# sebastian-hofstaetter/matchmaker

Hardware: NVIDIA H100
Metric: query-doc pairs scored/sec (ColBERT max-sim d=128) (higher is better)
Workload: dtype f16

## Files before the change

### matchmaker_b200/csrc/maxsim_qm.cu

```cuda
#include <cuda_bf16.h>
#include <cuda_fp16.h>

#include <algorithm>

#include "device_util.cuh"
#include "host_util.cuh"
#include "masks.cuh"
#include "maxsim.cuh"
#include "ptx.cuh"

namespace mmb {

namespace {

constexpr int kThreads = 384;
constexpr int kChunkRows = 64;
constexpr int kChunkKBlockBytes = kChunkRows * 128;
constexpr int kMaxStages = 32;
constexpr int kMaxLd = 4096;
constexpr int kScouts = 3;
constexpr int kRecordStep = 6;
constexpr int kMaxRecords = 48;
constexpr int kRecordReserve = 12 * 1024;
constexpr int kQSlots = 2;
constexpr int kQRows = 32;
constexpr int kQBlockBytes = kQRows * 128;
constexpr uint32_t kFill = 1u << 16, kLiveMask = kFill - 1;
constexpr int kRecBits = 4;
constexpr int kRegsHelper = 120, kRegsConsumer = 192;

#ifdef MMB200_ENABLE_PROF
enum QmProf {
  kPrTotal, kPrQEmpty, kPrRFull, kPrEmpty, kPrTma, kPrChunks,
  kCoTotal, kCoRFull, kCoFull, kCoIssue, kCoMma, kCoReduce, kCoEpilogue, kCoDocs,
  kScTotal, kScREmpty,
  kProfCount
};
__device__ unsigned long long g_qm_prof[kProfCount];
#define QM_PROF(...) __VA_ARGS__
#else
#define QM_PROF(...)
#endif

struct QmShared {
  uint64_t full[kMaxStages];
  uint64_t empty[kMaxStages];
  uint64_t qfull[kQSlots];
  uint64_t qempty[kQSlots];
  uint64_t rfull[kMaxRecords];
  uint64_t rempty[kMaxRecords];
  float xm[2][2][4][32];
  int32_t xa[2][2][4][32];
};

struct QmLaunch {
  int32_t kblocks;
  int32_t stages;
  int32_t chunk_bytes;
  int32_t records;
  int32_t rec_words;
};

struct RecCursor {
  int slot;
  uint32_t phase;
  __device__ __forceinline__ void advance(int step, int records) {
    slot += step;
    if (slot >= records) { slot -= records; phase ^= 1u; }
  }
};

struct QmMaps {
  CUtensorMap q;
  CUtensorMap d;
};

template <bool kStore>
struct PairStream {
  struct Batch {
    int32_t q, d, dm, rows;
    int64_t row0, row_end;
  };
  const MaxsimParams& P;
  int64_t first, end, step;
  int64_t pre_batch;
  int k;
  int lane;
  Batch cur, nxt, pre;

  __device__ __forceinline__ PairStream(const MaxsimParams& P_, int64_t first_, int64_t end_, int64_t step_, int lane_)
      : P(P_), first(first_), end(end_), step(step_), lane(lane_) {
    load1(cur, 0);
    load1(nxt, 1);
    load2(cur);
    load2(nxt);
    resolve(cur);
    pre_batch = 2;
    load1(pre, pre_batch);
    k = -1;
  }
  __device__ __forceinline__ void load1(Batch& b, int64_t bi) {
    const int64_t p = first + (bi * 32 + lane) * step;
    b.q = 0; b.d = -1; b.dm = 0; b.rows = 0; b.row0 = 0; b.row_end = 0;
    if (p >= end) return;
    b.q = P.pair_q ? P.pair_q[p] : (int32_t)((p + P.pair_base) / P.docs_per_query);
    b.d = P.pair_d ? P.pair_d[p] : (int32_t)p;
    if (P.pair_dmask) b.dm = P.pair_dmask[p];
  }
  __device__ __forceinline__ void load2(Batch& b) {
    if (!P.pair_dmask) b.dm = b.d;
    if constexpr (kStore) {
      if (b.d >= 0) { b.row0 = P.doc_offsets[b.d]; b.row_end = P.doc_offsets[b.d + 1]; }
    }
  }
  __device__ __forceinline__ void resolve(Batch& b) {
    if constexpr (kStore) b.rows = (int)max((int64_t)0, min(b.row_end - b.row0, (int64_t)P.Ld));
  }
  __device__ __forceinline__ void next() {
    if (++k == 32) {
      cur = nxt;
      resolve(cur);
      nxt = pre;
      load2(nxt);
      load1(pre, ++pre_batch);
      k = 0;
    }
  }
  __device__ __forceinline__ int64_t q() const { return __shfl_sync(0xffffffffu, cur.q, k); }
  __device__ __forceinline__ int64_t d() const { return __shfl_sync(0xffffffffu, cur.d, k); }
  __device__ __forceinline__ int64_t dm() const { return __shfl_sync(0xffffffffu, cur.dm, k); }
  __device__ __forceinline__ int rows() const { return __shfl_sync(0xffffffffu, cur.rows, k); }
  __device__ __forceinline__ int64_t row0() const { return __shfl_sync(0xffffffffu, cur.row0, k); }
};

template <typename T>
__device__ __forceinline__ void wgmma_n32(float (&d)[16], uint64_t a, uint64_t b, uint32_t acc);
template <>
__device__ __forceinline__ void wgmma_n32<__half>(float (&d)[16], uint64_t a, uint64_t b, uint32_t acc) {
  wgmma_m64n32k16_f16(d, a, b, acc);
}
template <>
__device__ __forceinline__ void wgmma_n32<__nv_bfloat16>(float (&d)[16], uint64_t a, uint64_t b, uint32_t acc) {
  wgmma_m64n32k16_bf16(d, a, b, acc);
}

template <bool kArgmax>
__device__ __forceinline__ void take(float v, int row, float& m, int& am) {
  if constexpr (kArgmax) {
    const bool gt = v > m;
    m = gt ? v : m;
    am = gt ? row : am;
  } else {
    m = fmaxf(m, v);
  }
}

template <typename T, bool kArgmax, bool kStore>
__global__ void __launch_bounds__(kThreads, 1)
maxsim_qm_kernel(const __grid_constant__ QmMaps M, MaxsimParams P, QmLaunch L) {
  extern __shared__ uint8_t smem_raw[];
  uint8_t* smem = smem_raw + ((1024u - (smem_u32(smem_raw) & 1023u)) & 1023u);
  const int qslot_bytes = L.kblocks * kQBlockBytes;
  uint8_t* q_base = smem;
  uint8_t* stage_base = q_base + kQSlots * qslot_bytes;
  uint32_t* rec_base = reinterpret_cast<uint32_t*>(stage_base + (size_t)L.stages * L.chunk_bytes);
  QmShared* S = reinterpret_cast<QmShared*>(rec_base + (size_t)L.records * L.rec_words);

  const int warp = threadIdx.x >> 5;
  const int lane = threadIdx.x & 31;

  int64_t p_begin, p_end;
  cta_share(P.n_pairs, &p_begin, &p_end);

  if (threadIdx.x == 0) {
    prefetch_tensormap(&M.q);
    prefetch_tensormap(&M.d);
    for (int s = 0; s < L.stages; ++s) { mbar_init(&S->full[s], 1); mbar_init(&S->empty[s], 4); }
    for (int s = 0; s < kQSlots; ++s) { mbar_init(&S->qfull[s], 1); mbar_init(&S->qempty[s], 8); }
    for (int r = 0; r < L.records; ++r) {
      mbar_init(&S->rfull[r], 1);
      mbar_init(&S->rempty[r], 5);
      rec_base[(size_t)r * L.rec_words + kRecBits - 2] = 0;
      rec_base[(size_t)r * L.rec_words + kRecBits - 1] = 0;
    }
    fence_barrier_init();
  }
  __syncthreads();

  if (warp == 0) {
    setmaxnreg_dec<kRegsHelper>();
    PairStream<kStore> meta(P, p_begin, p_end, 1, lane);
    const int ring = L.stages >> 1;
    int st_cur = 0, st_oth = 0;
    uint32_t ph_cur = 0, ph_oth = 0;
    int64_t prev_q = -1;
    uint32_t qcount = 0;
    RecCursor rc{0, 0};
    QM_PROF(unsigned long long prof[kProfCount] = {}; const long long t_start = clock64(); long long t_;)
    for (int64_t p = p_begin; p < p_end; ++p) {
      meta.next();
      const int64_t qi = meta.q();
      const int64_t di = meta.d();
      const int64_t row0 = kStore ? meta.row0() : 0;
      if (qi != prev_q) {
        const uint32_t slot = qcount & 1u, use = qcount >> 1;
        QM_PROF(t_ = clock64();)
        mbar_wait(&S->qempty[slot], (use & 1u) ^ 1u);
        QM_PROF(prof[kPrQEmpty] += clock64() - t_;)
        if (elect_one_sync()) {
          mbar_arrive_expect_tx(&S->qfull[slot], (uint32_t)(L.kblocks * kQBlockBytes));
          for (int kb = 0; kb < L.kblocks; ++kb)
            tma_load_4d(&M.q, q_base + (size_t)slot * qslot_bytes + kb * kQBlockBytes, &S->qfull[slot], 0, 0, kb, (int)qi,
                        kEvictLast);
        }
        __syncwarp();
        ++qcount;
        prev_q = qi;
      }
      const int c = (int)((p - p_begin) & 1);
      QM_PROF(t_ = clock64();)
      mbar_wait(&S->rfull[rc.slot], rc.phase);
      QM_PROF(prof[kPrRFull] += clock64() - t_;)
      const int live = (int)(rec_base[(size_t)rc.slot * L.rec_words] & kLiveMask);
      __syncwarp();
      if (lane == 0) mbar_arrive(&S->rempty[rc.slot]);
      rc.advance(1, L.records);
      const int dcoord = kStore ? 0 : (int)di;
      const int nch = max(1, (live + kChunkRows - 1) / kChunkRows);
      int row = kStore ? (int)row0 : live - kChunkRows * nch;
      for (int ch = 0; ch < nch; ++ch, row += kChunkRows) {
        const int stage = c * ring + st_cur;
        QM_PROF(t_ = clock64();)
        mbar_wait(&S->empty[stage], ph_cur ^ 1u);
        QM_PROF(prof[kPrEmpty] += clock64() - t_; t_ = clock64(); ++prof[kPrChunks];)
        if (elect_one_sync()) {
          if (live == 0) {
            mbar_arrive(&S->full[stage]);
          } else {
            mbar_arrive_expect_tx(&S->full[stage], (uint32_t)L.chunk_bytes);
            tma_load_4d(&M.d, stage_base + (size_t)stage * L.chunk_bytes, &S->full[stage], 0, row, 0, dcoord, kEvictFirst);
          }
        }
        __syncwarp();
        QM_PROF(prof[kPrTma] += clock64() - t_;)
        if (++st_cur == ring) { st_cur = 0; ph_cur ^= 1u; }
      }
      const int st = st_cur; st_cur = st_oth; st_oth = st;
      const uint32_t ph = ph_cur; ph_cur = ph_oth; ph_oth = ph;
    }
    QM_PROF(prof[kPrTotal] = clock64() - t_start;
            if (lane == 0) for (int i = kPrTotal; i <= kPrChunks; ++i) atomicAdd(&g_qm_prof[i], prof[i]);)
  } else if (warp <= kScouts) {
    setmaxnreg_dec<kRegsHelper>();
    constexpr int kW = 8;
    const int s = warp - 1;
    const int dmt = P.d_mask ? P.mask_dtype : MMB200_MASK_NONE;
    const int nwin = (P.Ld + 32 * kW - 1) / (32 * kW);
    const int bit_words = L.rec_words - kRecBits;
    PairStream<kStore> meta(P, p_begin + s, p_end, kScouts, lane);
    RecCursor rc{s, 0};
    int64_t fp = p_begin + s;
    auto load_win = [&](uint32_t (&raw)[kW], int64_t dm, int w) {
#pragma unroll
      for (int k = 0; k < kW; ++k) {
        const int g = w * 32 * kW + 32 * k + lane;
        raw[k] = 1;
        if (dmt != MMB200_MASK_NONE && g < P.Ld) {
          const uint64_t v = mask_raw(P.d_mask, dmt, dm * (int64_t)P.Ld + g);
          raw[k] = (uint32_t)(v | (v >> 32));
        }
      }
    };
    auto fetch = [&](uint32_t (&raw)[kW], int64_t& dm, int& lim) {
      if (fp < p_end) {
        meta.next();
        dm = meta.dm();
        lim = kStore ? meta.rows() : P.Ld;
        load_win(raw, dm, 0);
      }
      fp += kScouts;
    };
    QM_PROF(unsigned long long prof_re = 0; const long long t_start = clock64();)
    auto doc = [&](uint32_t (&raw)[kW], int64_t& dm, int& lim) {
      QM_PROF(const long long t_ = clock64();)
      mbar_wait(&S->rempty[rc.slot], rc.phase ^ 1u);
      QM_PROF(prof_re += clock64() - t_;)
      uint32_t* rec = rec_base + (size_t)rc.slot * L.rec_words;
      int live = 0;
      bool masked = false;
      for (int w = 0; w < nwin; ++w) {
        if (w > 0) load_win(raw, dm, w);
#pragma unroll
        for (int k = 0; k < kW; ++k) {
          const int g = w * 32 * kW + 32 * k + lane;
          const bool in_doc = g < lim;
          const bool ok = in_doc && mask_test(raw[k], dmt);
          masked |= in_doc && !ok;
          const uint32_t b = __ballot_sync(0xffffffffu, ok);
          const int wi = w * kW + k;
          if (b) live = 32 * wi + 32 - __clz(b);
          if (lane == 0 && wi < bit_words) rec[kRecBits + wi] = b;
        }
      }
      const bool fill = !kStore && __any_sync(0xffffffffu, masked);
      fetch(raw, dm, lim);
      if (lane == 0) {
        rec[0] = (uint32_t)live | (fill ? kFill : 0u);
        mbar_arrive(&S->rfull[rc.slot]);
      }
      rc.advance(kScouts, L.records);
    };
    uint32_t ra[kW], rb[kW];
    int64_t dma = 0, dmb = 0;
    int la = 0, lb = 0;
    fetch(ra, dma, la);
    fetch(rb, dmb, lb);
    for (int64_t sp = p_begin + s; sp < p_end;) {
      doc(ra, dma, la);
      if ((sp += kScouts) >= p_end) break;
      doc(rb, dmb, lb);
      sp += kScouts;
    }
    QM_PROF(if (lane == 0) {
      atomicAdd(&g_qm_prof[kScTotal], (unsigned long long)(clock64() - t_start));
      atomicAdd(&g_qm_prof[kScREmpty], prof_re);
    })
  } else {
    setmaxnreg_inc<kRegsConsumer>();
    const int c = (warp >> 2) - 1;
    const int wq = warp & 3;
    const int r0 = 16 * wq + (lane >> 2);
    const int qmt = P.q_mask ? P.mask_dtype : MMB200_MASK_NONE;
    const int ring = L.stages >> 1;
    int64_t prev_q = -1;
    uint32_t qcount = 0;
    int cur_slot = 0;
    RecCursor rc{c, 0};
    auto load_q = [&](int64_t n0) -> int32_t { return p_begin + n0 + lane < p_end ? P.pair_q[p_begin + n0 + lane] : 0; };
    int32_t qb_cur = 0, qb_nxt = 0;
    if (P.pair_q) { qb_cur = load_q(0); qb_nxt = load_q(32); }
    int64_t q_run = 0;
    int32_t q_rem = 0;
    if (!P.pair_q) {
      q_run = (p_begin + P.pair_base) / P.docs_per_query;
      q_rem = (int32_t)((p_begin + P.pair_base) - q_run * P.docs_per_query);
    }
    QM_PROF(unsigned long long prof[kProfCount] = {}; const long long t_start = clock64(); long long t_;)
    int64_t n_walk = 0;
    auto walk_to = [&](int64_t n) {
      for (; n_walk <= n; ++n_walk) {
        int64_t qi;
        if (P.pair_q) {
          if ((n_walk & 31) == 0 && n_walk > 0) { qb_cur = qb_nxt; qb_nxt = load_q(n_walk + 32); }
          qi = __shfl_sync(0xffffffffu, qb_cur, (int)(n_walk & 31));
        } else {
          qi = q_run;
          if (++q_rem == P.docs_per_query) { q_rem = 0; ++q_run; }
        }
        if (qi != prev_q) {
          if (prev_q >= 0) { __syncwarp(); if (lane == 0) mbar_arrive(&S->qempty[cur_slot]); }
          cur_slot = (int)(qcount & 1u);
          mbar_wait(&S->qfull[cur_slot], (qcount >> 1) & 1u);
          ++qcount;
          prev_q = qi;
        }
      }
      return prev_q;
    };
    struct Doc {
      int64_t n;
      uint32_t qlo;
      uint64_t qraw;
      int slot;
      uint32_t head;
      int live, nch;
    };
    auto begin = [&](Doc& D, int64_t n) {
      const int64_t qi = walk_to(n);
      D.n = n;
      D.qlo = (uint32_t)make_wgmma_sw128_desc(smem_u32(q_base + (size_t)cur_slot * qslot_bytes));
      D.qraw = 0;
      if (wq == 0 && lane < P.Lq)
        D.qraw = (qmt != MMB200_MASK_NONE) ? mask_raw(P.q_mask, qmt, qi * (int64_t)P.Lq + lane) : 1;
      QM_PROF(t_ = clock64();)
      mbar_wait(&S->rfull[rc.slot], rc.phase);
      QM_PROF(prof[kCoRFull] += clock64() - t_; ++prof[kCoDocs];)
      D.slot = rc.slot;
      rc.advance(2, L.records);
      D.head = rec_base[(size_t)D.slot * L.rec_words];
      D.live = (int)(D.head & kLiveMask);
      D.nch = max(1, (D.live + kChunkRows - 1) / kChunkRows);
    };
    int st_next = 0;
    uint32_t ph_next = 0;
    constexpr uint64_t kDescHi = (uint64_t)(1024 >> 4) << 32 | (uint64_t)1 << 62;
    auto issue = [&](float (&acc)[16], uint32_t qlo_doc) -> int {
      const int stage = c * ring + st_next;
      QM_PROF(t_ = clock64();)
      mbar_wait(&S->full[stage], ph_next);
      QM_PROF(prof[kCoFull] += clock64() - t_; t_ = clock64();)
      if (++st_next == ring) { st_next = 0; ph_next ^= 1u; }
      const uint32_t daddr = smem_u32(stage_base + (size_t)stage * L.chunk_bytes);
      const uint32_t dlo = (uint32_t)make_wgmma_sw128_desc(__shfl_sync(0xffffffffu, daddr, 0));
      const uint32_t qlo = __shfl_sync(0xffffffffu, qlo_doc, 0);
      wgmma_fence();
#pragma unroll
      for (int k = 0; k < 4; ++k) wgmma_n32<T>(acc, kDescHi | (dlo + 2 * k), kDescHi | (qlo + 2 * k), k != 0);
      if (L.kblocks > 1) {
#pragma unroll
        for (int k = 0; k < 4; ++k)
          wgmma_n32<T>(acc, kDescHi | (dlo + (kChunkKBlockBytes >> 4) + 2 * k),
                       kDescHi | (qlo + (kQBlockBytes >> 4) + 2 * k), 1);
      }
      wgmma_commit();
      wgmma_fence_regs(acc);
      QM_PROF(prof[kCoIssue] += clock64() - t_;)
      return stage;
    };
    float mx[8];
    int ax[8];
#pragma unroll
    for (int e = 0; e < 8; ++e) { mx[e] = -INFINITY; ax[e] = -1; }
    auto reduce = [&](float (&acc)[16], int stage, const Doc& D, int ch) {
      wgmma_fence_regs(acc);
      const int col0 = kStore ? kChunkRows * ch : D.live - kChunkRows * (D.nch - ch);
      const int x0 = col0 + r0, x1 = x0 + 8;
      const uint32_t* bits = rec_base + (size_t)D.slot * L.rec_words + kRecBits;
      const float p0 = (bits[x0 >> 5] >> (x0 & 31)) & 1u ? 0.f : -INFINITY;
      const float p1 = (bits[x1 >> 5] >> (x1 & 31)) & 1u ? 0.f : -INFINITY;
#pragma unroll
      for (int e = 0; e < 8; ++e) {
        const int i = 4 * (e >> 1) + (e & 1);
        take<kArgmax>(acc[i] + p0, x0, mx[e], ax[e]);
        take<kArgmax>(acc[i + 2] + p1, x1, mx[e], ax[e]);
      }
      __syncwarp();
      if (lane == 0) mbar_arrive(&S->empty[stage]);
    };
    auto combine = [&](float om, int oa, float& m, int& a) {
      if constexpr (kArgmax) {
        if (om > m || (om == m && (unsigned)oa < (unsigned)a)) { m = om; a = oa; }
      } else {
        m = fmaxf(m, om);
      }
    };
    auto epilogue = [&](const Doc& D) {
      QM_PROF(t_ = clock64();)
      if (lane == 0) mbar_arrive(&S->rempty[D.slot]);
#pragma unroll
      for (int o = 4; o < 32; o <<= 1) {
#pragma unroll
        for (int e = 0; e < 8; ++e) {
          const float om = __shfl_xor_sync(0xffffffffu, mx[e], o);
          const int oa = kArgmax ? __shfl_xor_sync(0xffffffffu, ax[e], o) : 0;
          combine(om, oa, mx[e], ax[e]);
        }
      }
      const int buf = (int)((D.n >> 1) & 1);
      float* xm = S->xm[c][buf][0];
      int32_t* xa = S->xa[c][buf][0];
      if (lane < 4) {
#pragma unroll
        for (int e = 0; e < 8; ++e) {
          const int t = 8 * (e >> 1) + 2 * lane + (e & 1);
          xm[32 * wq + t] = mx[e];
          if constexpr (kArgmax) xa[32 * wq + t] = ax[e];
        }
      }
#pragma unroll
      for (int e = 0; e < 8; ++e) { mx[e] = -INFINITY; ax[e] = -1; }
      if (wq != 0) {
        named_bar_arrive(1 + c, 128);
      } else {
        named_bar_sync(1 + c, 128);
        float m = xm[lane];
        int a = kArgmax ? xa[lane] : -1;
#pragma unroll
        for (int w = 1; w < 4; ++w) combine(xm[32 * w + lane], kArgmax ? xa[32 * w + lane] : 0, m, a);
        if (D.head & kFill) take<kArgmax>(-1000.f, P.Ld, m, a);
        const bool ok = mask_test(D.qraw, qmt);
        const int64_t p = p_begin + D.n;
        if constexpr (kArgmax) {
          if (lane < P.Lq) P.argmax[p * (int64_t)P.Lq + lane] = (ok && a < P.Ld) ? a : -1;
        }
        float s = ok ? m : 0.f;
        s += __shfl_down_sync(0xffffffffu, s, 8);
#pragma unroll
        for (int o = 1; o < 8; o <<= 1) s += __shfl_xor_sync(0xffffffffu, s, o);
        const float hi = __shfl_sync(0xffffffffu, s, 16);
        if (lane == 0) P.out[p] = s + hi;
      }
      QM_PROF(prof[kCoEpilogue] += clock64() - t_;)
    };
    const int64_t n_pairs = p_end - p_begin;
    float acc[16];
    for (int64_t n = c; n < n_pairs; n += 2) {
      Doc D;
      begin(D, n);
      for (int ch = 0; ch < D.nch; ++ch) {
        const int st = issue(acc, D.qlo);
        QM_PROF(t_ = clock64();)
        wgmma_wait<0>();
        QM_PROF(prof[kCoMma] += clock64() - t_; t_ = clock64();)
        reduce(acc, st, D, ch);
        QM_PROF(prof[kCoReduce] += clock64() - t_;)
      }
      epilogue(D);
    }
    QM_PROF(prof[kCoTotal] = clock64() - t_start;
            if (wq == 0 && lane == 0) for (int i = kCoTotal; i <= kCoDocs; ++i) atomicAdd(&g_qm_prof[i], prof[i]);)
  }
}

template <typename T, bool kArgmax, bool kStore>
int launch_qm(int grid, size_t smem_bytes, cudaStream_t stream, const QmMaps& M, const MaxsimParams& P,
              const QmLaunch& L) {
  MMB_CHECK_CUDA(cudaFuncSetAttribute(maxsim_qm_kernel<T, kArgmax, kStore>, cudaFuncAttributeMaxDynamicSharedMemorySize,
                                      (int)smem_bytes));
  maxsim_qm_kernel<T, kArgmax, kStore><<<grid, kThreads, smem_bytes, stream>>>(M, P, L);
  MMB_CHECK_CUDA(cudaGetLastError());
  return MMB200_OK;
}

int launch_qm_dispatch(int grid, size_t smem_bytes, cudaStream_t stream, const QmMaps& M, const MaxsimParams& P,
                       const QmLaunch& L, int dtype) {
  if (P.doc_offsets)
    return dtype == MMB200_F16 ? launch_qm<__half, false, true>(grid, smem_bytes, stream, M, P, L)
                               : launch_qm<__nv_bfloat16, false, true>(grid, smem_bytes, stream, M, P, L);
  if (dtype == MMB200_F16)
    return P.argmax ? launch_qm<__half, true, false>(grid, smem_bytes, stream, M, P, L)
                    : launch_qm<__half, false, false>(grid, smem_bytes, stream, M, P, L);
  return P.argmax ? launch_qm<__nv_bfloat16, true, false>(grid, smem_bytes, stream, M, P, L)
                  : launch_qm<__nv_bfloat16, false, false>(grid, smem_bytes, stream, M, P, L);
}

}

int maxsim_qm_launch(const MaxsimParams& P, int dtype, const DeviceInfo& dev, cudaStream_t stream, bool* handled) {
  *handled = false;
  if (dtype != MMB200_F16 && dtype != MMB200_BF16) return MMB200_OK;
  if (P.Lq > kQRows || (P.dim != 64 && P.dim != 128) || P.Ld > kMaxLd) return MMB200_OK;
  if ((reinterpret_cast<uintptr_t>(P.q) | reinterpret_cast<uintptr_t>(P.d)) & 15) return MMB200_OK;
  if (P.doc_offsets && P.argmax) return MMB200_OK;
  QmLaunch L;
  L.kblocks = P.dim / 64;
  L.chunk_bytes = L.kblocks * kChunkKBlockBytes;
  L.rec_words = kRecBits + 2 * ((P.Ld + kChunkRows - 1) / kChunkRows);
  const int fixed = kQSlots * L.kblocks * kQBlockBytes + (int)sizeof(QmShared) + 1024;
  L.stages = std::min(kMaxStages, (dev.max_smem_optin - fixed - kRecordReserve) / L.chunk_bytes) & ~1;
  const int rec_bytes = L.rec_words * 4;
  L.records = std::min(kMaxRecords, (dev.max_smem_optin - fixed - L.stages * L.chunk_bytes) / rec_bytes);
  L.records -= L.records % kRecordStep;
  if (L.stages < 4 || L.records < kRecordStep) return MMB200_OK;
  const size_t smem_bytes = (size_t)L.stages * L.chunk_bytes + (size_t)L.records * rec_bytes + fixed;

  const CUtensorMapDataType tdt = dtype == MMB200_F16 ? CU_TENSOR_MAP_DATA_TYPE_FLOAT16 : CU_TENSOR_MAP_DATA_TYPE_BFLOAT16;
  QmMaps M;
  {
    const uint64_t dims[4] = {64, (uint64_t)P.Lq, (uint64_t)L.kblocks, (uint64_t)P.n_q};
    const uint64_t strides[3] = {(uint64_t)P.dim * 2, 128, (uint64_t)P.Lq * P.dim * 2};
    const uint32_t box[4] = {64, (uint32_t)kQRows, 1, 1};
    if (int rc = encode_tensor_map(&M.q, tdt, 4, P.q, dims, strides, box, CU_TENSOR_MAP_SWIZZLE_128B,
                                   CU_TENSOR_MAP_L2_PROMOTION_L2_128B))
      return rc;
  }
  const uint64_t d_rows = P.doc_offsets ? (uint64_t)P.n_rows : (uint64_t)P.Ld;
  const uint64_t d_count = P.doc_offsets ? 1 : (uint64_t)P.n_d;
  {
    const uint64_t dims[4] = {64, d_rows, (uint64_t)L.kblocks, d_count};
    const uint64_t strides[3] = {(uint64_t)P.dim * 2, 128, d_rows * P.dim * 2};
    const uint32_t box[4] = {64, (uint32_t)kChunkRows, (uint32_t)L.kblocks, 1};
    if (int rc = encode_tensor_map(&M.d, tdt, 4, P.d, dims, strides, box, CU_TENSOR_MAP_SWIZZLE_128B,
                                   CU_TENSOR_MAP_L2_PROMOTION_L2_256B))
      return rc;
  }
  *handled = true;
  const int grid = (int)std::min<int64_t>(dev.sm_count, P.n_pairs);
#ifdef MMB200_ENABLE_PROF
  const bool prof = getenv("MMB200_MAXSIM_PROF") != nullptr;
  if (prof) {
    const unsigned long long zero[kProfCount] = {};
    MMB_CHECK_CUDA(cudaMemcpyToSymbolAsync(g_qm_prof, zero, sizeof(zero), 0, cudaMemcpyHostToDevice, stream));
  }
  const int rc = launch_qm_dispatch(grid, smem_bytes, stream, M, P, L, dtype);
  if (prof && rc == MMB200_OK) {
    unsigned long long h[kProfCount];
    MMB_CHECK_CUDA(cudaMemcpyFromSymbolAsync(h, g_qm_prof, sizeof(h), 0, cudaMemcpyDeviceToHost, stream));
    MMB_CHECK_CUDA(cudaStreamSynchronize(stream));
    const double ctas = grid, wgs = 2.0 * grid, scouts = (double)kScouts * grid;
    const double chunks = (double)h[kPrChunks], docs = (double)h[kCoDocs];
    fprintf(stderr,
            "maxsim_prof pairs %lld Ld %d chunks %.0f | cycles per CTA: producer total %.0f qempty %.0f rfull %.0f "
            "empty %.0f tma %.0f | per consumer warpgroup: total %.0f rfull %.0f full %.0f issue %.0f mma %.0f "
            "reduce %.0f epilogue %.0f | per scout: total %.0f rempty %.0f | per chunk: producer %.0f (empty %.0f, "
            "tma %.0f), warpgroup full %.0f issue %.0f mma %.0f reduce %.0f | per document per warpgroup: total %.0f "
            "epilogue %.0f rfull %.0f\n",
            (long long)P.n_pairs, P.Ld, chunks, h[kPrTotal] / ctas, h[kPrQEmpty] / ctas, h[kPrRFull] / ctas,
            h[kPrEmpty] / ctas, h[kPrTma] / ctas, h[kCoTotal] / wgs, h[kCoRFull] / wgs, h[kCoFull] / wgs,
            h[kCoIssue] / wgs, h[kCoMma] / wgs, h[kCoReduce] / wgs, h[kCoEpilogue] / wgs, h[kScTotal] / scouts,
            h[kScREmpty] / scouts, h[kPrTotal] / chunks, h[kPrEmpty] / chunks, h[kPrTma] / chunks, h[kCoFull] / chunks,
            h[kCoIssue] / chunks, h[kCoMma] / chunks, h[kCoReduce] / chunks, h[kCoTotal] / docs, h[kCoEpilogue] / docs,
            h[kCoRFull] / docs);
  }
  return rc;
#else
  return launch_qm_dispatch(grid, smem_bytes, stream, M, P, L, dtype);
#endif
}

}
```

Before: 145.6 million.

## Use three consumer warpgroups instead of two in maxsim kernel

Raises the CTA from 384 to 512 threads so three consumer warpgroups take pairs round-robin. The stage ring is split three ways, the producer rotates over three stage cursors, and record stepping and barrier counts are adjusted to match. The intent is more concurrent MMA and reduction work per SM to hide epilogue and wait latency. In exchange, consumer registers drop from 192 to 128 per thread and there are fewer stages per consumer ring, which could cause spills or starve the pipeline.

```diff
diff --git a/matchmaker_b200/csrc/maxsim_qm.cu b/matchmaker_b200/csrc/maxsim_qm.cu
--- a/matchmaker_b200/csrc/maxsim_qm.cu
+++ b/matchmaker_b200/csrc/maxsim_qm.cu
@@ -13,27 +13,29 @@
 
 namespace {
 
-constexpr int kThreads = 384;
+constexpr int kThreads = 512;
+constexpr int kConsumers = 3;
 constexpr int kChunkRows = 64;
 constexpr int kChunkKBlockBytes = kChunkRows * 128;
-constexpr int kMaxStages = 32;
+constexpr int kMaxStages = 30;
 constexpr int kMaxLd = 4096;
 constexpr int kScouts = 3;
-constexpr int kRecordStep = 6;
+constexpr int kRecordStep = 3;
 constexpr int kMaxRecords = 48;
-constexpr int kRecordReserve = 12 * 1024;
+constexpr int kRecordReserve = 10 * 1024;
 constexpr int kQSlots = 2;
 constexpr int kQRows = 32;
 constexpr int kQBlockBytes = kQRows * 128;
 constexpr uint32_t kFill = 1u << 16, kLiveMask = kFill - 1;
 constexpr int kRecBits = 4;
-constexpr int kRegsHelper = 120, kRegsConsumer = 192;
+constexpr int kRegsHelper = 128, kRegsConsumer = 128;
 
 #ifdef MMB200_ENABLE_PROF
 enum QmProf {
   kPrTotal, kPrQEmpty, kPrRFull, kPrEmpty, kPrTma, kPrChunks,
   kCoTotal, kCoRFull, kCoFull, kCoIssue, kCoMma, kCoReduce, kCoEpilogue, kCoDocs,
   kScTotal, kScREmpty,
+  kPrMaxChunks, kCoMaxTotal,
   kProfCount
 };
 __device__ unsigned long long g_qm_prof[kProfCount];
@@ -49,8 +51,8 @@
   uint64_t qempty[kQSlots];
   uint64_t rfull[kMaxRecords];
   uint64_t rempty[kMaxRecords];
-  float xm[2][2][4][32];
-  int32_t xa[2][2][4][32];
+  float xm[kConsumers][2][4][32];
+  int32_t xa[kConsumers][2][4][32];
 };
 
 struct QmLaunch {
@@ -176,7 +178,7 @@
     prefetch_tensormap(&M.q);
     prefetch_tensormap(&M.d);
     for (int s = 0; s < L.stages; ++s) { mbar_init(&S->full[s], 1); mbar_init(&S->empty[s], 4); }
-    for (int s = 0; s < kQSlots; ++s) { mbar_init(&S->qfull[s], 1); mbar_init(&S->qempty[s], 8); }
+    for (int s = 0; s < kQSlots; ++s) { mbar_init(&S->qfull[s], 1); mbar_init(&S->qempty[s], 4 * kConsumers); }
     for (int r = 0; r < L.records; ++r) {
       mbar_init(&S->rfull[r], 1);
       mbar_init(&S->rempty[r], 5);
@@ -190,9 +192,10 @@
   if (warp == 0) {
     setmaxnreg_dec<kRegsHelper>();
     PairStream<kStore> meta(P, p_begin, p_end, 1, lane);
-    const int ring = L.stages >> 1;
-    int st_cur = 0, st_oth = 0;
-    uint32_t ph_cur = 0, ph_oth = 0;
+    const int ring = L.stages / kConsumers;
+    int c = 0;
+    int st_cur = 0, st_n1 = 0, st_n2 = 0;
+    uint32_t ph_cur = 0, ph_n1 = 0, ph_n2 = 0;
     int64_t prev_q = -1;
     uint32_t qcount = 0;
     RecCursor rc{0, 0};
@@ -217,7 +220,6 @@
         ++qcount;
         prev_q = qi;
       }
-      const int c = (int)((p - p_begin) & 1);
       QM_PROF(t_ = clock64();)
       mbar_wait(&S->rfull[rc.slot], rc.phase);
       QM_PROF(prof[kPrRFull] += clock64() - t_;)
@@ -245,11 +247,15 @@
         QM_PROF(prof[kPrTma] += clock64() - t_;)
         if (++st_cur == ring) { st_cur = 0; ph_cur ^= 1u; }
       }
-      const int st = st_cur; st_cur = st_oth; st_oth = st;
-      const uint32_t ph = ph_cur; ph_cur = ph_oth; ph_oth = ph;
+      const int st = st_cur; st_cur = st_n1; st_n1 = st_n2; st_n2 = st;
+      const uint32_t ph = ph_cur; ph_cur = ph_n1; ph_n1 = ph_n2; ph_n2 = ph;
+      if (++c == kConsumers) c = 0;
     }
     QM_PROF(prof[kPrTotal] = clock64() - t_start;
-            if (lane == 0) for (int i = kPrTotal; i <= kPrChunks; ++i) atomicAdd(&g_qm_prof[i], prof[i]);)
+            if (lane == 0) {
+              for (int i = kPrTotal; i <= kPrChunks; ++i) atomicAdd(&g_qm_prof[i], prof[i]);
+              atomicMax(&g_qm_prof[kPrMaxChunks], prof[kPrChunks]);
+            })
   } else if (warp <= kScouts) {
     setmaxnreg_dec<kRegsHelper>();
     constexpr int kW = 8;
@@ -331,7 +337,7 @@
     const int wq = warp & 3;
     const int r0 = 16 * wq + (lane >> 2);
     const int qmt = P.q_mask ? P.mask_dtype : MMB200_MASK_NONE;
-    const int ring = L.stages >> 1;
+    const int ring = L.stages / kConsumers;
     int64_t prev_q = -1;
     uint32_t qcount = 0;
     int cur_slot = 0;
@@ -386,7 +392,7 @@
       mbar_wait(&S->rfull[rc.slot], rc.phase);
       QM_PROF(prof[kCoRFull] += clock64() - t_; ++prof[kCoDocs];)
       D.slot = rc.slot;
-      rc.advance(2, L.records);
+      rc.advance(kConsumers, L.records);
       D.head = rec_base[(size_t)D.slot * L.rec_words];
       D.live = (int)(D.head & kLiveMask);
       D.nch = max(1, (D.live + kChunkRows - 1) / kChunkRows);
@@ -444,6 +450,7 @@
         m = fmaxf(m, om);
       }
     };
+    int xbuf = 0;
     auto epilogue = [&](const Doc& D) {
       QM_PROF(t_ = clock64();)
       if (lane == 0) mbar_arrive(&S->rempty[D.slot]);
@@ -456,9 +463,9 @@
           combine(om, oa, mx[e], ax[e]);
         }
       }
-      const int buf = (int)((D.n >> 1) & 1);
-      float* xm = S->xm[c][buf][0];
-      int32_t* xa = S->xa[c][buf][0];
+      float* xm = S->xm[c][xbuf][0];
+      int32_t* xa = S->xa[c][xbuf][0];
+      xbuf ^= 1;
       if (lane < 4) {
 #pragma unroll
         for (int e = 0; e < 8; ++e) {
@@ -494,7 +501,7 @@
     };
     const int64_t n_pairs = p_end - p_begin;
     float acc[16];
-    for (int64_t n = c; n < n_pairs; n += 2) {
+    for (int64_t n = c; n < n_pairs; n += kConsumers) {
       Doc D;
       begin(D, n);
       for (int ch = 0; ch < D.nch; ++ch) {
@@ -507,8 +514,12 @@
       }
       epilogue(D);
     }
+    walk_to(n_pairs - 1);
     QM_PROF(prof[kCoTotal] = clock64() - t_start;
-            if (wq == 0 && lane == 0) for (int i = kCoTotal; i <= kCoDocs; ++i) atomicAdd(&g_qm_prof[i], prof[i]);)
+            if (wq == 0 && lane == 0) {
+              for (int i = kCoTotal; i <= kCoDocs; ++i) atomicAdd(&g_qm_prof[i], prof[i]);
+              atomicMax(&g_qm_prof[kCoMaxTotal], prof[kCoTotal]);
+            })
   }
 }
 
@@ -547,11 +558,12 @@
   L.chunk_bytes = L.kblocks * kChunkKBlockBytes;
   L.rec_words = kRecBits + 2 * ((P.Ld + kChunkRows - 1) / kChunkRows);
   const int fixed = kQSlots * L.kblocks * kQBlockBytes + (int)sizeof(QmShared) + 1024;
-  L.stages = std::min(kMaxStages, (dev.max_smem_optin - fixed - kRecordReserve) / L.chunk_bytes) & ~1;
+  L.stages = std::min(kMaxStages, (dev.max_smem_optin - fixed - kRecordReserve) / L.chunk_bytes);
+  L.stages -= L.stages % kConsumers;
   const int rec_bytes = L.rec_words * 4;
   L.records = std::min(kMaxRecords, (dev.max_smem_optin - fixed - L.stages * L.chunk_bytes) / rec_bytes);
   L.records -= L.records % kRecordStep;
-  if (L.stages < 4 || L.records < kRecordStep) return MMB200_OK;
+  if (L.stages < 2 * kConsumers || L.records < kRecordStep) return MMB200_OK;
   const size_t smem_bytes = (size_t)L.stages * L.chunk_bytes + (size_t)L.records * rec_bytes + fixed;
 
   const CUtensorMapDataType tdt = dtype == MMB200_F16 ? CU_TENSOR_MAP_DATA_TYPE_FLOAT16 : CU_TENSOR_MAP_DATA_TYPE_BFLOAT16;
@@ -587,20 +599,20 @@
     unsigned long long h[kProfCount];
     MMB_CHECK_CUDA(cudaMemcpyFromSymbolAsync(h, g_qm_prof, sizeof(h), 0, cudaMemcpyDeviceToHost, stream));
     MMB_CHECK_CUDA(cudaStreamSynchronize(stream));
-    const double ctas = grid, wgs = 2.0 * grid, scouts = (double)kScouts * grid;
+    const double ctas = grid, wgs = (double)kConsumers * grid, scouts = (double)kScouts * grid;
     const double chunks = (double)h[kPrChunks], docs = (double)h[kCoDocs];
     fprintf(stderr,
             "maxsim_prof pairs %lld Ld %d chunks %.0f | cycles per CTA: producer total %.0f qempty %.0f rfull %.0f "
             "empty %.0f tma %.0f | per consumer warpgroup: total %.0f rfull %.0f full %.0f issue %.0f mma %.0f "
             "reduce %.0f epilogue %.0f | per scout: total %.0f rempty %.0f | per chunk: producer %.0f (empty %.0f, "
             "tma %.0f), warpgroup full %.0f issue %.0f mma %.0f reduce %.0f | per document per warpgroup: total %.0f "
-            "epilogue %.0f rfull %.0f\n",
+            "epilogue %.0f rfull %.0f | slowest consumer warpgroup: total %.0f | most chunks of a CTA %.0f\n",
             (long long)P.n_pairs, P.Ld, chunks, h[kPrTotal] / ctas, h[kPrQEmpty] / ctas, h[kPrRFull] / ctas,
             h[kPrEmpty] / ctas, h[kPrTma] / ctas, h[kCoTotal] / wgs, h[kCoRFull] / wgs, h[kCoFull] / wgs,
             h[kCoIssue] / wgs, h[kCoMma] / wgs, h[kCoReduce] / wgs, h[kCoEpilogue] / wgs, h[kScTotal] / scouts,
             h[kScREmpty] / scouts, h[kPrTotal] / chunks, h[kPrEmpty] / chunks, h[kPrTma] / chunks, h[kCoFull] / chunks,
             h[kCoIssue] / chunks, h[kCoMma] / chunks, h[kCoReduce] / chunks, h[kCoTotal] / docs, h[kCoEpilogue] / docs,
-            h[kCoRFull] / docs);
+            h[kCoRFull] / docs, (double)h[kCoMaxTotal], (double)h[kPrMaxChunks]);
   }
   return rc;
 #else
```

After: 147.2 million (median of 6 runs). 1.01x the previous value.
